# CarminLiu/ORB_SLAM2_aruco

Hardware: AMD Instinct MI355X
Metric: frames/s (ORB+ArUco extract+match, 640x480 mono) (higher is better)
Workload: dtype u8

## Files before the change

orb_slam2_aruco_amd/csrc/aruco_detector.hip:

```cpp
#include <algorithm>
#include <array>
#include <cmath>
#include <cstdlib>
#include <functional>
#include <limits>
#include <map>

#include "aruco_kernels.hpp"
#include "aruco_pose.hpp"
#include "detector_plan.hpp"
#include "host_stage.hpp"
#include "orbfe_common.hpp"
#include "orbfe_tables.inc"

using namespace orbfe;

struct ModeRun {
    const uint8_t* d_full = nullptr;
    size_t full_fstride = 0, full_step = 0;
    int full_rows = 0, full_cols = 0;
    int fixed_thr = -1;
    uint32_t* d_hist = nullptr;
    std::function<int(hipStream_t)> before_finalize;
};
// ... 10 lines not shown
struct DetectorQueues {
    hipStream_t own_stream = nullptr, aux_stream = nullptr;
    hipEvent_t ev_fork = nullptr, ev_join = nullptr;
    ~DetectorQueues()
    {
        if (own_stream) (void)hipStreamDestroy(own_stream);
        if (aux_stream) (void)hipStreamDestroy(aux_stream);
        if (ev_fork) (void)hipEventDestroy(ev_fork);
        if (ev_join) (void)hipEventDestroy(ev_join);
    }
};

struct orbfe_aruco : DetectorQueues {
    int device = 0;
    std::string dict_name;
    int nbits = 0, nb = 0, S = 0, ncodes = 0;
    hipStream_t user_aux = nullptr;
    DetectorSwitches sw;
    DetectorGeometry geo;
    int batch_cap = 0;
    DevBuf d_twork, d_trect, d_tctr;
    DevBuf d_rstate, d_lut;
    DevBuf d_segs, d_tailkeys, d_tailoff, d_small, d_hint;
    PinnedBuf pinned;
    DevBuf d_poses;
    struct Spec {
        bool pending = false, has_pose = false;
        int rows = 0, cols = 0;
        const uint8_t* host_copy = nullptr;
        size_t host_pitch = 0;
        PoseCamera cam{};
        float size = 0.f;
    } spec;
    bool last_cam_valid = false;
    PoseCamera last_cam{};
    float last_size = 0.f;
    DevBuf d_dwork, d_dctr, d_ditems, d_dhist, d_dpatch;
    bool decode_dirty = false;
    bool tail_dirty = false;
    int n_escalations = 0;
    DevBuf d_ctmlist;
    bool ct_dirty = true;
    unsigned ct_gen = 0;
    bool ct_tab_dirty = true;
    DevBuf d_ctseg, d_cthtab, d_ctelem, d_ctstate, d_ctitemsA, d_ctitemsB, d_ctnitems, d_ctcodes;
    DevBuf d_tstrips, d_ttabs, d_ttab2;
    ThresholdTables ttab;
    template <class T> static int upload(DevBuf& d, const std::vector<T>& v)
    {
        if (int rc = d.ensure(v.size() * sizeof(T))) return rc;
        if (!v.empty()) ORBFE_HIP(hipMemcpy(d.p, v.data(), v.size() * sizeof(T), hipMemcpyHostToDevice));
        return ORBFE_OK;
    }
    int ensure_threshold_tables()
    {
        if (ttab.cols == geo.cols && ttab.win == geo.win) return ORBFE_OK;
        ThresholdTables fresh = plan_threshold_tables(geo.cols, geo.win);
        ttab = ThresholdTables{};
        if (!fresh.ok) return fail(ORBFE_ERR_INVALID, "matrix-core threshold tables refused a %d-pixel row at window %d", geo.cols, geo.win);
        int rc;
        if ((rc = upload(d_tstrips, fresh.strips)) || (rc = upload(d_ttabs, fresh.tabs)) || (rc = upload(d_ttab2, fresh.tab2))) return rc;
        ttab = std::move(fresh);
        return ORBFE_OK;
    }
    bool specks_ran = false;
    DevBuf d_bitsc;
    DevBuf d_codes, d_levels, d_bits, d_pyr, d_candq, d_pool, d_kept, d_rects, d_counts, d_candidx, d_ncand,
        d_result, d_gpad;
    DevBuf d_in, d_out, d_nout;
    float error_rate = 0.0f;
    int max_corr = 0, tau = 0, nsorted = 0;
    int corner_method = 1;
    DevBuf d_scodes, d_sids, d_msrc;
    int detect_mode = 0;
    int thres_method = 0;
    int thres_value = 7;
    int n_attempts_auto_fix = 3;
    float min_size = 0.f;
    bool auto_size = false;
    float ts = 0.25f;
    bool enclosed = false;
    int tracking_min = 0;
    std::map<int, int> marker_counts;
    std::vector<orbfe_marker> prev_markers;
    int last_tracked = 0;
    int gray_bits15 = 0;
    int last_attempts = 0, last_work_rows = 0, last_work_cols = 0;
    size_t rl_static = 0;
    DevBuf d_red, d_mhist, d_masks, d_bgr, d_bits2;
    template <class Batch> int with_retries(Batch&& batch, const int32_t* counts, int nframes)
    {
        for (Contours floor = Contours::tiled;;) {
            Contours ran = Contours::none; int flags_or = 0, rc;
            if ((rc = batch(floor, &ran))) return rc;
            ORBFE_HIP(hipStreamSynchronize(own_stream));
            for (int f = 0; f < nframes; f++) flags_or |= counts[f * 4 + 2];
            if (sw.force_legacy || (floor = escalate(ran, flags_or, geo.relay_tbits != 0)) == Contours::none) return ORBFE_OK;
            n_escalations++;
        }
    }
    bool stateful() const { return thres_method == 1 || auto_size || tracking_min > 0; }
    KernelTimer timer;
    int last_nframes = 0;

    int set_dictionary(const char* name)
    {
        for (int i = 0; i < ORBFE_NDICTS; i++)
            if (!strcmp(ORBFE_DICTS[i].name, name)) {
                const orbfe_dict_entry& d = ORBFE_DICTS[i];
                if (d.nbits > 36) return fail(ORBFE_ERR_DICT, "dictionary %s: %d-bit codes are not supported", name, d.nbits);
// ... 156 lines not shown
        decode_dirty = false;
        return ORBFE_OK;
    }

    ImgView pyr_view() { return ImgView{d_pyr.as<uint8_t>(), d_pyr.as<uint8_t>(), geo.pyr_fbytes, 0}; }
    void pyramid(int first, const ImgView& src0, int B, hipStream_t st)
    {
        const ImgView pyr = pyr_view();
        const std::vector<PyrKernel> K = plan_pyramid_kernels(geo, first, (unsigned)((uintptr_t)src0.base & 15), src0.pitch, src0.fstride, sw.half_pyr);
        if (first == 1 && first < geo.npyr && (K[1] == PyrKernel::half_pyr4 || K[1] == PyrKernel::half_pyr3)) {
            const int nf = K[1] == PyrKernel::half_pyr4 ? 4 : 3, bs = 1 << nf;
            HalfPyrDst P{};
            P.base = pyr.base_w; P.fstride = geo.pyr_fbytes;
            for (int p = 1; p <= nf; p++) { P.off[p - 1] = (uint32_t)geo.levels[p].off; P.pitch[p - 1] = geo.levels[p].pitch; }
            const int bw = geo.levels[0].w / bs, nblocks = bw * (geo.levels[0].h / bs);
            if (nf == 4) hipLaunchKernelGGL(k_half_pyr<4>, dim3((nblocks + 255) / 256, B), dim3(256), 0, st, src0, P, bw, nblocks);
            else hipLaunchKernelGGL(k_half_pyr<3>, dim3((nblocks + 255) / 256, B), dim3(256), 0, st, src0, P, bw, nblocks);
            first = nf + 1;
        }
        for (int p = first; p < geo.npyr; p++) {
            const ArLevel &L = geo.levels[p], &Lp = geo.levels[p - 1];
            ImgView sv = (p == 1) ? src0 : ImgView{pyr.base + Lp.off, nullptr, geo.pyr_fbytes, Lp.pitch};
            ImgView dv{pyr.base + L.off, pyr.base_w + L.off, geo.pyr_fbytes, L.pitch};
            if (K[p] == PyrKernel::half_area4) {
                const int dw4 = (L.w + 3) / 4, nthreads = dw4 * ((L.h + 1) / 2);
                hipLaunchKernelGGL(k_half_area4, dim3((nthreads + 255) / 256, B), dim3(256), 0, st, sv, dv, dw4, L.h);
            } else if (K[p] == PyrKernel::half_area) {
                hipLaunchKernelGGL(k_half_area, dim3((L.w + 63) / 64, (L.h + 3) / 4, B), dim3(256), 0, st, sv, dv, L.w, L.h);
            } else {
                const int dw4 = (L.w + 3) / 4;
                const double scale_x = 1. / ((double)L.w / Lp.w), scale_y = 1. / ((double)L.h / Lp.h);
                hipLaunchKernelGGL(k_resize_level, dim3((dw4 + 63) / 64, (L.h + 7) / 8, B), dim3(256), 0, st, sv, dv,
                                   Lp.w, Lp.h, dw4, L.h, scale_x, scale_y, L.w);
            }
        }
    }
    template <class K> K by_window(K k5, K k7, K k11, K k15) const { return geo.win == 5 ? k5 : geo.win == 7 ? k7 : geo.win == 11 ? k11 : k15; }
    int threshold(const BatchPlan& p, const ImgView& srcW, const ImgView& src0, int fixed_thr, int B, hipStream_t s, int* enlarge_k)
    {
        for (int r_ = 0; r_ < ORBFE_REPS_ARUCO(8); r_++) {
            const int ntx = (geo.cols + 63) / 64, ntl = ntx * ((geo.rows + 63) / 64);
            const dim3 tg(ntx, (geo.rows + 63) / 64, B), tg1(xcd_grid(ntl * B));
            uint32_t* bp = d_bits.as<uint32_t>();
            if (p.thr == Thr::fixed) {
                if (enclosed) {
                    if (int rc = d_bits2.ensure(geo.bits_fu32 * 4 * B)) return rc;
                    const int k = *enlarge_k = int(std::max(3.0, 3. / 1920. * float(geo.cols))) | 1;
                    if (k / 2 > 15) return fail(ORBFE_ERR_INVALID, "detectEnclosedMarkers: frame too wide (erosion size %d)", k);
                }
                hipLaunchKernelGGL(k_fixed_threshold, dim3((geo.wpr * geo.rows + 255) / 256, B), dim3(256), 0, s, srcW, geo.cols, geo.rows, fixed_thr, enclosed ? d_bits2.as<uint32_t>() : bp, geo.bits_fu32, geo.wpr);
                if (enclosed) hipLaunchKernelGGL(k_erode_cross_xor, dim3((geo.wpr * geo.rows + 255) / 256, B), dim3(256), 0, s, d_bits2.as<uint32_t>(), bp, geo.bits_fu32, geo.wpr, geo.cols, geo.rows, *enlarge_k / 2);
            } else if (p.thr == Thr::mfma) {
                const int n2 = geo.win * geo.win, n_tstrips = (int)ttab.strips.size(), nxs = (n_tstrips + 3) / 4;
                hipLaunchKernelGGL(k_threshold_mfma, dim3(xcd_grid(nxs * B)), dim3(256), 0, s, srcW, geo.cols, geo.rows, ttab.rb, -(n2 * thres_value - n2 / 2),
                                   d_tstrips.as<ThrStrip>(), d_ttabs.as<uint4>(), d_ttab2.as<uint4>(), bp, geo.bits_fu32, geo.wpr, n_tstrips, nxs, nxs * B, n2 > 127 ? 1 : 0);
            } else if (p.thr == Thr::pyr) {
                ThrPyr P{};
                P.n = p.nfuse;
                for (int l = 1; l <= p.nfuse; l++) { P.w[l - 1] = geo.levels[l].w; P.h[l - 1] = geo.levels[l].h; P.pitch[l - 1] = geo.levels[l].pitch; P.off[l - 1] = geo.levels[l].off; }
                hipLaunchKernelGGL(by_window(k_threshold_pyr<5>, k_threshold_pyr<7>, k_threshold_pyr<11>, k_threshold_pyr<15>), tg1, dim3(256), 0, s,
                                   srcW, geo.cols, geo.rows, p.thr_kk, bp, geo.bits_fu32, geo.wpr, ntx, ntl, ntl * B, pyr_view(), P);
                if (p.nfuse && r_ == 0) pyramid(p.nfuse + 1, src0, B, s);
            } else if (geo.win <= 15) hipLaunchKernelGGL(k_adaptive_threshold<7>, tg, dim3(256), 0, s, srcW, geo.cols, geo.rows, geo.win, thres_value, 1.0 / (geo.win * geo.win), bp, geo.bits_fu32, geo.wpr);
            else hipLaunchKernelGGL(k_adaptive_threshold<15>, tg, dim3(256), 0, s, srcW, geo.cols, geo.rows, geo.win, thres_value, 1.0 / (geo.win * geo.win), bp, geo.bits_fu32, geo.wpr);
        }
        return ORBFE_OK;
    }
    int speck_pass(const BatchPlan& p, int B, hipStream_t s)
    {
        int rc;
        const size_t spk_lds = speck_lds_bytes(geo.cols);
        if (!(specks_ran = p.specks)) return ORBFE_OK;
        if ((rc = d_bitsc.ensure(geo.bits_fu32 * 4 * batch_cap)) || (rc = ensure_dyn_lds(reinterpret_cast<const void*>(k_speck_clean), spk_lds))) return rc;
        hipLaunchKernelGGL(k_speck_clean, dim3((geo.rows + SPK_ROWS - 1) / SPK_ROWS, B), dim3(SPK_THREADS), spk_lds, s, d_bits.as<uint32_t>(), geo.bits_fu32, geo.wpr,
                           geo.cols, geo.rows, d_bitsc.as<uint32_t>());
        return ORBFE_OK;
    }
    int contours_tiled(const BatchPlan& p, int B, const uint32_t* cbits, hipStream_t s)
    {
        int rc;
        const int cw = p.tile_w, ncols = (geo.cols + cw - 1) / cw, nbands = (geo.rows + 31) / 32, total_tiles = ncols * nbands * B;
        const int wave_bytes = ctw_wave_lds_bytes(cw), wlds = wave_bytes * (CTW_THREADS / 64);
        const int walk_wgs = std::max(1, std::min((total_tiles / p.tpw + CTW_THREADS / 64 - 1) / (CTW_THREADS / 64), 256 * 8));
        const size_t llds = (size_t)geo.ct_lcap * 8 + 16;
        if ((rc = ensure_dyn_lds(reinterpret_cast<const void*>(k_ct_walk), (size_t)wlds)) || (rc = ensure_dyn_lds(reinterpret_cast<const void*>(k_ct_lists), llds))) return rc;
        if (ct_dirty) ORBFE_HIP(hipMemsetAsync(d_ctstate.p, 0, (size_t)CT_STATE_INTS * 4 * B, s));
        ct_gen = (ct_gen + 1) & 0xffffu;
        if (ct_gen == 0) { ct_gen = 1; ct_tab_dirty = true; }
        if (ct_tab_dirty) { ORBFE_HIP(hipMemsetAsync(d_cthtab.p, 0, d_cthtab.bytes, s)); ct_tab_dirty = false; }
        ct_dirty = true;
        if (p.band) {
            const int nb = ((geo.rows + 31) / 32 + p.band_rows - 1) / p.band_rows;
            const size_t blds = ctb_lds_bytes(geo.cols, p.band_rows);
            if ((rc = ensure_dyn_lds(reinterpret_cast<const void*>(k_ct_band), blds))) return rc;
            hipLaunchKernelGGL(k_ct_band, dim3(nb, B), dim3(CTB_THREADS), blds, s, cbits, geo.bits_fu32, geo.wpr, geo.cols, geo.rows, 70,
                               d_lut.as<uint16_t>(), p.band_rows, d_ctmlist.as<uint32_t>(), CTB_MCAP, d_cthtab.as<unsigned long long>(), geo.ct_hbits, ct_gen,
                               d_ctseg.as<uint32_t>(), (size_t)5 * geo.ct_segcap, geo.ct_segcap, d_ctstate.as<int32_t>(), d_pool.as<uint32_t>(), geo.pool_fu32,
                               (int)geo.pool_fu32, geo.relay_kcap, d_tailkeys.as<unsigned long long>(), d_tailoff.as<int32_t>(), d_ctcodes.as<uint4>());
        } else
            hipLaunchKernelGGL(k_ct_walk, dim3(walk_wgs), dim3(CTW_THREADS), wlds, s, cbits, geo.bits_fu32, geo.wpr, geo.cols, geo.rows, 70,
                               d_lut.as<uint16_t>(), cw, ncols, nbands, total_tiles, d_cthtab.as<unsigned long long>(), geo.ct_hbits, ct_gen,
                               d_ctseg.as<uint32_t>(), (size_t)5 * geo.ct_segcap, geo.ct_segcap, d_ctstate.as<int32_t>(), d_pool.as<uint32_t>(), geo.pool_fu32,
                               (int)geo.pool_fu32, geo.relay_kcap, d_tailkeys.as<unsigned long long>(), d_tailoff.as<int32_t>(), wave_bytes,
                               d_ctcodes.as<uint4>());
        hipLaunchKernelGGL(k_ct_lists, dim3(B), dim3(geo.ct_lcap > 4096 ? 1024 : 512), llds, s, d_ctseg.as<uint32_t>(), (size_t)5 * geo.ct_segcap, geo.ct_segcap,
                           d_ctstate.as<int32_t>(), d_cthtab.as<unsigned long long>(), geo.ct_hbits, ct_gen, d_ctelem.as<unsigned long long>(), geo.ct_lcap, 70,
                           (int)geo.pool_fu32, geo.relay_kcap, d_tailkeys.as<unsigned long long>(), d_tailoff.as<int32_t>(), d_counts.as<int32_t>(),
// ... 1029 lines not shown
```

orb_slam2_aruco_amd/csrc/aruco_kernels.hip:

```cpp
#include "aruco_kernels.hpp"
#include "wave_dpp.hpp"

#ifndef ORBFE_PRIO_DET_TAIL
#define ORBFE_PRIO_DET_TAIL 0
#endif
namespace orbfe {

__device__ __forceinline__ int a_lane_prefix(unsigned long long mask)
{
    return __builtin_amdgcn_mbcnt_hi((unsigned)(mask >> 32), __builtin_amdgcn_mbcnt_lo((unsigned)mask, 0));
}

__device__ __forceinline__ uint32_t bl_dot4_a(uint32_t a, uint32_t b, uint32_t c) { return __builtin_amdgcn_udot4(a, b, c, false); }

template <int TH_MAXR>
__global__ __launch_bounds__(256) void k_adaptive_threshold(ImgView src, int W, int H, int win, int C, double scale,
                                                            uint32_t* __restrict__ bits, size_t bits_fstride, int wpr)
{
    constexpr int TH_NLD = (16 + 2 * TH_MAXR + 3) / 4;
    __shared__ uint8_t sin[16 + 2 * TH_MAXR][64 + 2 * TH_MAXR + 2];
    __shared__ uint16_t sh[16 + 2 * TH_MAXR][64];
    const int r = win >> 1;
    const int tx0 = blockIdx.x * 64, tyb = blockIdx.y * 64, f = blockIdx.z;
    const int tid = threadIdx.x, lane = tid & 63, wid = tid >> 6;
// ... 177 lines not shown
        }
    }
    if (P.n >= 1) {
        uint8_t* pf = pyr.base_w + (size_t)f * pyr.fstride;
        {
            const int j = tid >> 3, d = tid & 7;
            const uint2 a0 = *reinterpret_cast<const uint2*>(&spx[2 * j][2 * d]), a1 = *reinterpret_cast<const uint2*>(&spx[2 * j + 1][2 * d]);
            const uint32_t o = th_half4(a0, a1);
            l1[j][d] = o;
            const int y = (ty0 >> 1) + j, x = (tx0 >> 1) + 4 * d;
            if (y < P.h[0] && x < P.w[0]) *reinterpret_cast<uint32_t*>(pf + P.off[0] + (uint32_t)(__mul24(y, P.pitch[0]) + x)) = o;
        }
        if (P.n >= 2) {
            __syncthreads();
            if (tid < 64) {
                const int j = tid >> 2, d = tid & 3;
                const uint2 a0 = *reinterpret_cast<const uint2*>(&l1[2 * j][2 * d]), a1 = *reinterpret_cast<const uint2*>(&l1[2 * j + 1][2 * d]);
                const uint32_t o = th_half4(a0, a1);
                l2[j][d] = o;
                const int y = (ty0 >> 2) + j, x = (tx0 >> 2) + 4 * d;
                if (y < P.h[1] && x < P.w[1]) *reinterpret_cast<uint32_t*>(pf + P.off[1] + (uint32_t)(__mul24(y, P.pitch[1]) + x)) = o;
            }
        }
        if (P.n >= 3) {
            __syncthreads();
            if (tid < 16) {
                const int j = tid >> 1, d = tid & 1;
                const uint2 a0 = *reinterpret_cast<const uint2*>(&l2[2 * j][2 * d]), a1 = *reinterpret_cast<const uint2*>(&l2[2 * j + 1][2 * d]);
                const uint32_t o = th_half4(a0, a1);
                l3[j][d] = o;
                const int y = (ty0 >> 3) + j, x = (tx0 >> 3) + 4 * d;
                if (y < P.h[2] && x < P.w[2]) *reinterpret_cast<uint32_t*>(pf + P.off[2] + (uint32_t)(__mul24(y, P.pitch[2]) + x)) = o;
            }
        }
        if (P.n >= 4) {
            __syncthreads();
            if (tid < 4) {
                const int j = tid;
                const uint2 a0 = *reinterpret_cast<const uint2*>(&l3[2 * j][0]), a1 = *reinterpret_cast<const uint2*>(&l3[2 * j + 1][0]);
                const uint32_t o = th_half4(a0, a1);
                const int y = (ty0 >> 4) + j, x = tx0 >> 4;
                if (y < P.h[3] && x < P.w[3]) *reinterpret_cast<uint32_t*>(pf + P.off[3] + (uint32_t)(__mul24(y, P.pitch[3]) + x)) = o;
            }
        }
    }
}
template __global__ void k_threshold_pyr<5>(ImgView, int, int, uint32_t, uint32_t*, size_t, int, int, int, int, ImgView, ThrPyr);
template __global__ void k_threshold_pyr<7>(ImgView, int, int, uint32_t, uint32_t*, size_t, int, int, int, int, ImgView, ThrPyr);
template __global__ void k_threshold_pyr<11>(ImgView, int, int, uint32_t, uint32_t*, size_t, int, int, int, int, ImgView, ThrPyr);
template __global__ void k_threshold_pyr<15>(ImgView, int, int, uint32_t, uint32_t*, size_t, int, int, int, int, ImgView, ThrPyr);

typedef int tm_v4i __attribute__((ext_vector_type(4)));
typedef int tm_v16i __attribute__((ext_vector_type(16)));
__global__ __launch_bounds__(256) void k_threshold_mfma(ImgView src, int W, int H, int rb , int kinit,
                                                        const ThrStrip* __restrict__ strips, const uint4* __restrict__ tabs,
                                                        const uint4* __restrict__ tab2, uint32_t* __restrict__ bits, size_t bits_fstride,
                                                        int wpr, int nstrips, int nx, int total, int two_centre)
{
    const int lane = threadIdx.x & 63, wid = threadIdx.x >> 6;
    int bx, f;
    if (!xcd_remap(nx, total, bx, f)) return;
    const int si = bx * 4 + wid;
    if (si >= nstrips) return;
    const ThrStrip S = strips[si];
    const int r = lane & 31, half = lane >> 5;
    const uint8_t* img = src.base + (size_t)f * src.fstride;
    const tm_v4i Ba = __builtin_bit_cast(tm_v4i, tabs[(size_t)S.tab * 64 + lane]), Bb = __builtin_bit_cast(tm_v4i, tabs[(size_t)(S.tab + 1) * 64 + lane]);
    const tm_v4i Ia = __builtin_bit_cast(tm_v4i, tabs[(size_t)(S.tab + 2) * 64 + lane]), Ib = __builtin_bit_cast(tm_v4i, tabs[(size_t)(S.tab + 3) * 64 + lane]);
    const tm_v4i V2a = __builtin_bit_cast(tm_v4i, tab2[lane]), V2b = __builtin_bit_cast(tm_v4i, tab2[64 + lane]);
    const tm_v4i C2a = __builtin_bit_cast(tm_v4i, tab2[128 + lane]), C2b = __builtin_bit_cast(tm_v4i, tab2[192 + lane]);
    const tm_v4i C3a = __builtin_bit_cast(tm_v4i, tab2[256 + lane]), C3b = __builtin_bit_cast(tm_v4i, tab2[320 + lane]);
    const uint32_t ca = (uint32_t)(half ? S.c1 : S.c0), cb = (uint32_t)S.c2;
    typedef uint32_t tm_u32x4 __attribute__((ext_vector_type(4)));
    typedef tm_u32x4 tm_u32x4_unaligned __attribute__((aligned(1)));
    const int nblk = ((H + 31) >> 5) + 1;
    auto load_rows = [&](int j, tm_u32x4& pa, tm_u32x4& pb) {
        const uint32_t ro = (uint32_t)__mul24(min(max(32 * j - rb + r, 0), H - 1), src.pitch);
        pa = *reinterpret_cast<const tm_u32x4_unaligned*>(img + (ro + ca));
        pb = *reinterpret_cast<const tm_u32x4_unaligned*>(img + (ro + cb));
    };
    tm_u32x4 na, nb;
    load_rows(0, na, nb);
    const tm_v16i c128 = {128, 128, 128, 128, 128, 128, 128, 128, 128, 128, 128, 128, 128, 128, 128, 128};
    const tm_v16i ckin = {kinit, kinit, kinit, kinit, kinit, kinit, kinit, kinit, kinit, kinit, kinit, kinit, kinit, kinit, kinit, kinit};
    const tm_v16i czero = {0, 0, 0, 0, 0, 0, 0, 0, 0, 0, 0, 0, 0, 0, 0, 0};
    tm_v4i ph = {0, 0, 0, 0}, pl = {0, 0, 0, 0}, pc = {0, 0, 0, 0};
    const uint32_t valid = (S.x0 + 32 <= W) ? 0xffffffffu : ((1u << (W - S.x0)) - 1u);
    uint32_t* brow = bits + (size_t)f * bits_fstride + (S.x0 >> 5);
    for (int j = 0; j < nblk; j++) {
        const tm_u32x4 qa = na, qb = nb;
        if (j + 1 < nblk) load_rows(j + 1, na, nb);
        constexpr uint32_t SGN = 0x80808080u;
        const tm_v4i A1a = {(int)(qa.x ^ SGN), (int)(qa.y ^ SGN), (int)(qa.z ^ SGN), (int)(qa.w ^ SGN)};
        const tm_v4i A1b = {(int)(qb.x ^ SGN), (int)(qb.y ^ SGN), (int)(qb.z ^ SGN), (int)(qb.w ^ SGN)};
        tm_v16i acc = __builtin_amdgcn_mfma_i32_32x32x32_i8(A1a, Ba, c128, 0, 0, 0);
        tm_v16i sel = __builtin_amdgcn_mfma_i32_32x32x32_i8(A1a, Ia, czero, 0, 0, 0);
        acc = __builtin_amdgcn_mfma_i32_32x32x32_i8(A1b, Bb, acc, 0, 0, 0);
        sel = __builtin_amdgcn_mfma_i32_32x32x32_i8(A1b, Ib, sel, 0, 0, 0);
        tm_v4i nh, nl, nc;
#pragma unroll
        for (int q = 0; q < 4; q++) {
            const uint32_t a0 = (uint32_t)acc[4 * q], a1 = (uint32_t)acc[4 * q + 1], a2 = (uint32_t)acc[4 * q + 2], a3 = (uint32_t)acc[4 * q + 3];
            nh[q] = (int)(__builtin_amdgcn_perm(a1, a0, 0x0c0c0501u) | __builtin_amdgcn_perm(a3, a2, 0x05010c0cu));
            nl[q] = (int)((__builtin_amdgcn_perm(a1, a0, 0x0c0c0400u) | __builtin_amdgcn_perm(a3, a2, 0x04000c0cu)) ^ SGN);
            const uint32_t c0 = (uint32_t)sel[4 * q], c1 = (uint32_t)sel[4 * q + 1], c2 = (uint32_t)sel[4 * q + 2], c3 = (uint32_t)sel[4 * q + 3];
            nc[q] = (int)(__builtin_amdgcn_perm(c1, c0, 0x0c0c0400u) | __builtin_amdgcn_perm(c3, c2, 0x04000c0cu));
        }
        if (j >= 1) {
            tm_v16i ah = __builtin_amdgcn_mfma_i32_32x32x32_i8(ph, V2a, czero, 0, 0, 0);
            tm_v16i al = __builtin_amdgcn_mfma_i32_32x32x32_i8(pl, V2a, ckin, 0, 0, 0);
            ah = __builtin_amdgcn_mfma_i32_32x32x32_i8(nh, V2b, ah, 0, 0, 0);
            al = __builtin_amdgcn_mfma_i32_32x32x32_i8(nl, V2b, al, 0, 0, 0);
            al = __builtin_amdgcn_mfma_i32_32x32x32_i8(pc, C2a, al, 0, 0, 0);
            al = __builtin_amdgcn_mfma_i32_32x32x32_i8(nc, C2b, al, 0, 0, 0);
            if (two_centre) {
                al = __builtin_amdgcn_mfma_i32_32x32x32_i8(pc, C3a, al, 0, 0, 0);
                al = __builtin_amdgcn_mfma_i32_32x32x32_i8(nc, C3b, al, 0, 0, 0);
            }
            uint32_t wbits = 0;
#pragma unroll
            for (int q = 0; q < 4; q++) {
                uint32_t t4[4];
#pragma unroll
                for (int k = 0; k < 4; k++) t4[k] = ((uint32_t)ah[4 * q + k] << 8) + (uint32_t)al[4 * q + k];
                const uint32_t sg = (__builtin_amdgcn_perm(t4[1], t4[0], 0x0c0c0703u) | __builtin_amdgcn_perm(t4[3], t4[2], 0x07030c0cu)) & SGN;
                const uint32_t nib = (sg * 0x00204081u) >> 28;
                wbits |= nib << (8 * q);
            }
            wbits <<= 4 * half;
            wbits |= (uint32_t)__shfl_xor((int)wbits, 32);
            const int y = 32 * (j - 1) + r;
            if (half == 0 && y < H) brow[(uint32_t)__mul24(y, wpr)] = ~wbits & valid;
        }
        ph = nh; pl = nl; pc = nc;
    }
}

template <int WW, int HH>
__device__ __forceinline__ void speck_pass_lds(uint32_t* P, uint32_t* Fm, uint32_t* Sm, uint32_t* An, int NR, int PWS, int tid)
{
    const int n = NR * PWS;
    const float inv_pws = 1.0f / (float)PWS;
    for (int i = tid; i < n; i += SPK_THREADS) {
        const int r = (int)(((float)i + 0.5f) * inv_pws), j = i - __mul24(r, PWS);
        uint32_t f = 0, sd = 0;
        if (j + 1 < PWS) speck_row_masks<WW>(P[i], P[i + 1], &f, &sd);
        Fm[i] = f; Sm[i] = sd;
    }
    __syncthreads();
    for (int i = tid; i < n; i += SPK_THREADS) {
        const int r = (int)(((float)i + 0.5f) * inv_pws);
        uint32_t a = 0;
        if (r + HH + 1 < NR) {
            uint32_t occ = Fm[i] | Fm[i + (HH + 1) * PWS];
#pragma unroll
            for (int k = 1; k <= HH; k++) occ |= Sm[i + k * PWS];
            a = ~occ;
        }
        An[i] = a;
    }
    __syncthreads();
    for (int i = tid; i < n; i += SPK_THREADS) {
        const int r = (int)(((float)i + 0.5f) * inv_pws), j = i - __mul24(r, PWS);
        if (r < HH) continue;
        uint32_t e = 0, el = 0;
#pragma unroll
        for (int dy = 1; dy <= HH; dy++) {
            e |= An[i - dy * PWS];
            if (j) el |= An[i - dy * PWS - 1];
        }
        P[i] &= ~speck_dilate<WW>(e, el);
    }
    __syncthreads();
}

__global__ __launch_bounds__(SPK_THREADS) void k_speck_clean(const uint32_t* __restrict__ bits, size_t bits_fstride, int wpr_g, int W, int H,
                                                             uint32_t* __restrict__ out)
{
    extern __shared__ __align__(16) uint32_t spk_smem[];
    constexpr int RCH = ORBFE_SPECK_REACH, NR = SPK_ROWS + 2 * RCH;
    const int tid = threadIdx.x, f = blockIdx.y, y0 = blockIdx.x * SPK_ROWS;
    const int pw = (W + 2 + 31) >> 5, PWS = pw + 1, n = NR * PWS;
    uint32_t* P = spk_smem;
    uint32_t* Fm = P + n;
    uint32_t* Sm = Fm + n;
    uint32_t* An = Sm + n;
    const uint32_t* gb = bits + (size_t)f * bits_fstride;
    const float inv_pws = 1.0f / (float)PWS;
    for (int i = tid; i < n; i += SPK_THREADS) {
// ... 2358 lines not shown
```

orb_slam2_aruco_amd/csrc/aruco_kernels.hpp:

```cpp
#pragma once
#include <hip/hip_runtime.h>
#include <stdint.h>

#include "aruco_trace.hpp"
#include "detector_plan.hpp"
#include "orb_kernels.hpp"

namespace orbfe {

#define AR_MAX_RECTS 256

struct ArKept {
    int off, len;
    short vx[4], vy[4];
};
struct ArRect {
    float c[4][2];
    int off, len;
};

template <int TH_MAXR>
__global__ void k_adaptive_threshold(ImgView src, int W, int H, int win, int C, double scale, uint32_t* bits,
                                     size_t bits_fstride, int wpr);
__global__ void k_threshold_mfma(ImgView src, int W, int H, int rb, int kinit, const ThrStrip* strips, const uint4* tabs, const uint4* tab2,
                                 uint32_t* bits, size_t bits_fstride, int wpr, int nstrips, int nx, int total, int two_centre);
struct ThrPyr { int n; int w[4], h[4], pitch[4]; long long off[4]; };
template <int WIN>
__global__ void k_threshold_pyr(ImgView src, int W, int H, uint32_t kk, uint32_t* bits, size_t bits_fstride, int wpr, int ntx, int ntiles,
                                int total, ImgView pyr, ThrPyr P);
#ifndef ORBFE_CAND_FILTER
#define ORBFE_CAND_FILTER 1
#endif
__global__ void k_speck_clean(const uint32_t* bits, size_t bits_fstride, int wpr_g, int W, int H, uint32_t* out);
__global__ void k_half_area(ImgView src, ImgView dst, int dw, int dh);
__global__ void k_half_area4(ImgView src, ImgView dst, int dw4, int dh);
struct HalfPyrDst { uint8_t* base; size_t fstride; uint32_t off[4]; int pitch[4]; };
template <int NF> __global__ void k_half_pyr(ImgView src, HalfPyrDst P, int bw, int nblocks);
template <bool LDS_BITS>
__global__ void k_contours_t(const uint32_t* gbits, size_t bits_fstride, int wpr_g, int W, int H, int lds_bits_words,
                           int min_len, uint32_t* candq, size_t candq_fstride, int candq_cap, uint32_t* pool,
                           size_t pool_fstride, int pool_cap, ArKept* kept_out, int kept_cap, ArRect* rects_out,
                           int rect_cap, int32_t* counts, uint32_t* gpadded, size_t gpadded_fstride, int only_flagged);

struct RelaySeg {
    uint32_t nxt;
    uint32_t len;
    uint32_t minoff;
    uint32_t stg;
    uint32_t mn;
};
__global__ void k_contours_relay(const uint32_t* gbits, size_t bits_fstride, int wpr_g, int W, int H,
                                 int lds_bits_words, int min_len, int kshift, int tbits, RelaySeg* segs, uint32_t* pool,
                                 size_t pool_fstride, int pool_cap, ArKept* kept_out, int kept_cap, int kcap,
                                 unsigned long long* tail_keys, int32_t* tail_off, int32_t* counts, int32_t* hint, uint4* small_g, int32_t* rstate, int small_elsewhere, const uint16_t* lut_g, int f0, uint32_t* candq_g, size_t candq_fstride);
__global__ void k_contours_relay8(const uint32_t* gbits, size_t bits_fstride, int wpr_g, int W, int H,
                                 int lds_bits_words, int min_len, int kshift, int tbits, RelaySeg* segs, uint32_t* pool,
                                 size_t pool_fstride, int pool_cap, ArKept* kept_out, int kept_cap, int kcap,
                                 unsigned long long* tail_keys, int32_t* tail_off, int32_t* counts, int32_t* hint, uint4* small_g, int32_t* rstate, int small_elsewhere, const uint16_t* lut_g, int f0, uint32_t* candq_g, size_t candq_fstride);
__global__ void k_contours_relay_wide(const uint32_t* gbits, size_t bits_fstride, int wpr_g, int W, int H,
                                 int lds_bits_words, int min_len, int kshift, int tbits, RelaySeg* segs, uint32_t* pool,
                                 size_t pool_fstride, int pool_cap, ArKept* kept_out, int kept_cap, int kcap,
                                 unsigned long long* tail_keys, int32_t* tail_off, int32_t* counts, int32_t* hint, uint4* small_g, int32_t* rstate, int small_elsewhere, const uint16_t* lut_g, int f0, uint32_t* candq_g, size_t candq_fstride);
__global__ void k_contours_relay8g(const uint32_t* gbits, size_t bits_fstride, int wpr_g, int W, int H,
                                 int lds_bits_words, int min_len, int kshift, int tbits, RelaySeg* segs, uint32_t* pool,
                                 size_t pool_fstride, int pool_cap, ArKept* kept_out, int kept_cap, int kcap,
                                 unsigned long long* tail_keys, int32_t* tail_off, int32_t* counts, int32_t* hint, uint4* small_g, int32_t* rstate,
                                 uint32_t* gpad, size_t gpad_fstride, const uint16_t* lut_g, int f0);
__global__ void k_relay_lut(uint16_t* lut);
__global__ void k_contours_small(const uint32_t* gbits, size_t bits_fstride, int wpr_g, int W, int H, int min_len, const uint16_t* lut_g,
                                 int32_t* rstate, uint32_t* pool, size_t pool_fstride, int pool_cap, int kcap, unsigned long long* tail_keys,
                                 int32_t* tail_off, int32_t* counts);
__global__ void k_tail_prep(const unsigned long long* tail_keys, const int32_t* tail_off, int kcap, const int32_t* counts, uint4* work, size_t work_half,
                            int32_t* ctr);
__global__ void k_tail_approx(int kcap, const uint4* work, size_t work_half, const int32_t* ctr, const uint32_t* pool, size_t pool_fstride, ArKept* kept_out,
                              int kept_cap, uint8_t* rectflag, int pts);
__global__ void k_tail_finish(int kcap, const uint8_t* rectflag, const ArKept* kept_out, int kept_cap, ArRect* rects_out, int rect_cap,
// ... 121 lines not shown
```

orb_slam2_aruco_amd/csrc/detector_plan.hpp:

```cpp
#pragma once
#include <stddef.h>
#include <stdint.h>

#include <algorithm>
#include <cstdarg>
#include <cstdio>
#include <cstdlib>
#include <vector>

#include "../../include/orbfe.h"
#include "aruco_trace.hpp"
#include "input_layout.hpp"

namespace orbfe {

#define AR_MAX_KEPT 1024
#define AR_MAX_KEPT_BIG 4096
#define RL_KCAP AR_MAX_KEPT
#define CTW_MAX_CW 480
#define AR_FLAG_KEPT 2
#define AR_FLAG_POOL 4
#define AR_CAPACITY_FLAGS (AR_FLAG_KEPT | AR_FLAG_POOL)
#define RL_FLAG_TABLE 32
#define RL_FLAG_BUG 64
// ... 111 lines not shown
    const bool large = (size_t)rows * cols > (size_t)640 * 480 * 3 / 2;
    if (g.lds_bits_words && large && relay_lds_bytes(g.lds_bits_words, RL_KCAP, 13) + rl_static <= 160 * 1024) g.relay_tbits = 13;
    else if (g.lds_bits_words && relay_lds_bytes(g.lds_bits_words, RL_KCAP, 12) + rl_static <= 160 * 1024) g.relay_tbits = 12;
    g.relay_global = !g.relay_tbits && relay_lds_bytes(0, AR_MAX_KEPT_BIG, 13) + rl_static <= 160 * 1024;
    if (g.relay_global) { g.relay_tbits = 13; g.relay_kcap = AR_MAX_KEPT_BIG; }
    int sc = 4096;
    while (sc < rows * cols / 32 && sc < 65536) sc <<= 1;
    g.ct_segcap = std::min(sc, 65535);
    g.ct_hbits = 1;
    while ((1 << g.ct_hbits) < 2 * sc) g.ct_hbits++;
    g.ct_lcap = std::min(g.ct_segcap, lcap_override > 0 ? lcap_override : large ? 16384 : 4096);
    g.ct_items_per_frame = std::max(4096, g.ct_segcap / 4);
    return g;
}

enum class PyrKernel : int { none = 0, half_pyr4, half_pyr3, half_area4, half_area, resize_level };

inline std::vector<PyrKernel> plan_pyramid_kernels(const DetectorGeometry& geo, int first, unsigned src_align, int src_pitch, size_t src_fstride, bool half_pyr)
{
    std::vector<PyrKernel> k((size_t)std::max(geo.npyr, 0), PyrKernel::none);
    if (first == 1 && half_pyr)
        for (int nf = 4; nf >= 3 && first == 1; nf--) {
            const int bs = 1 << nf, al0 = bs == 16 ? 16 : 8;
            bool ok = geo.npyr > nf && geo.levels[0].w % bs == 0 && geo.levels[0].h % bs == 0 && src_pitch % al0 == 0 && src_fstride % al0 == 0 &&
                      (src_align & (unsigned)(al0 - 1)) == 0 && geo.pyr_fbytes % 8 == 0;
            for (int p = 1; ok && p <= nf; p++) {
                const int al = bs >> p;
                ok = geo.lvl_exact[p] && geo.levels[p].w == geo.levels[0].w >> p && geo.levels[p].h == geo.levels[0].h >> p && geo.levels[p].pitch % al == 0 &&
                     geo.levels[p].off % al == 0 && geo.levels[p].pitch >= geo.levels[p].w;
            }
            if (!ok) continue;
            for (int p = 1; p <= nf; p++) k[(size_t)p] = nf == 4 ? PyrKernel::half_pyr4 : PyrKernel::half_pyr3;
            first = nf + 1;
        }
    for (int p = std::max(first, 1); p < geo.npyr; p++) {
        const ArLevel &L = geo.levels[(size_t)p], &Lp = geo.levels[(size_t)p - 1];
        const bool own = p > 1;
        const int spitch = own ? Lp.pitch : src_pitch;
        const size_t sfstride = own ? geo.pyr_fbytes : src_fstride;
        const unsigned salign = own ? (unsigned)(Lp.off & 15) : src_align;
        if (!geo.lvl_exact[(size_t)p]) k[(size_t)p] = PyrKernel::resize_level;
        else if (spitch % 8 == 0 && sfstride % 8 == 0 && (salign & 7) == 0 && L.pitch % 4 == 0 && L.pitch >= 4 * ((L.w + 3) / 4)) k[(size_t)p] = PyrKernel::half_area4;
        else k[(size_t)p] = PyrKernel::half_area;
    }
    return k;
}

struct ThrStrip { int x0, c0, c1, c2, tab; };

struct ThresholdTables {
    int cols = 0, win = 0;
    bool ok = false;
    int rb = 0;
    std::vector<ThrStrip> strips;
    std::vector<uint8_t> tabs, tab2;
};

inline bool threshold_tables_apply(int cols, int win) { return win / 2 <= 7 && cols >= 48; }

inline ThresholdTables plan_threshold_tables(int cols, int win)
{
    ThresholdTables t;
    t.cols = cols; t.win = win;
    const int R = win / 2, n2 = win * win, W = cols, rb = R <= 3 ? 4 : 8;
    if (!threshold_tables_apply(cols, win)) return t;
    t.tabs.reserve((size_t)(W + 31) / 32 * 4096);
    for (int X = 0; X < W; X += 32) {
        ThrStrip S{};
        S.x0 = X; S.tab = (int)(t.tabs.size() / 1024);
        auto cl = [&](int c) { return std::min(std::max(c, 0), W - 16); };
        S.c0 = cl(X - rb); S.c1 = cl(X - rb + 16); S.c2 = cl(X - rb + 32);
        const int cs[3] = {S.c0, S.c1, S.c2};
        auto owner = [&](int x) {
            for (int pz = 0; pz < 3; pz++)
                if (x >= cs[pz] && x < cs[pz] + 16) return pz;
            return -1;
        };
        const size_t base = t.tabs.size();
        t.tabs.resize(base + 4096, 0);
        auto entry = [&](int m, int n, int piece, int x) -> uint8_t& {
            return t.tabs[base + (size_t)(m + (piece == 2)) * 1024 + (size_t)(n + 32 * (piece == 1)) * 16 + (x - cs[piece])];
        };
        for (int n = 0; n < 32 && X + n < W; n++) {
            for (int u = -R; u <= R; u++) {
                const int x = std::min(std::max(X + n + u, 0), W - 1), piece = owner(x);
                if (piece < 0) return t;
                entry(0, n, piece, x) += 1;
            }
            entry(2, n, owner(X + n), X + n) = 1;
        }
        t.strips.push_back(S);
    }
    t.tab2.assign(6144, 0);
    const int cw1 = n2 <= 127 ? n2 : 113, cw2 = n2 - cw1;
    for (int m = 0; m < 6; m++)
        for (int lane = 0; lane < 64; lane++) {
            const int n = lane & 31, half = lane >> 5;
            for (int i = 0; i < 16; i++) {
                const int q = 4 * half + (i & 3) + 8 * (i >> 2);
                const int d = ((m & 1) ? 32 : 0) + q - rb - n;
                int v = 0;
                if (m < 2) v = (d >= -R && d <= R) ? 1 : 0;
                else v = d == 0 ? -(m < 4 ? cw1 : cw2) : 0;
                t.tab2[(size_t)m * 1024 + (size_t)lane * 16 + i] = (uint8_t)(int8_t)v;
            }
        }
    t.rb = rb;
    t.ok = true;
    return t;
}

struct DetectorSwitches {
    int tiled = -1;
    int banded = -1;
    int band_rows = 0;
    int tile_w = 0;
    int tpw = 0;
    int lcap = 0;
    int specks = -1;
    bool specks_inkernel = false;
    bool relay_wide = true;
    int small_separate = -1;
    bool thr_mfma = true;
    bool thr_mfma_auto = true;
    bool thr_pyr = true;
    bool half_pyr = true;
    bool force_legacy = false;
    bool big_mode = false;
};

typedef const char* (*EnvLookup)(const char* name);
inline void read_detector_env(DetectorSwitches& sw, EnvLookup env)
{
    auto num = [&](const char* name, int unset) { const char* v = env(name); return v ? atoi(v) : unset; };
    auto tri = [&](const char* name, int unset) { const char* v = env(name); return v ? (atoi(v) ? 1 : 0) : unset; };
    sw.relay_wide = num("ORBFE_ARUCO_RELAY_WIDE", 1) != 0;
    sw.small_separate = num("ORBFE_ARUCO_SMALL_SEPARATE", sw.small_separate);
    sw.tiled = tri("ORBFE_ARUCO_TILED", sw.tiled);
    sw.banded = tri("ORBFE_ARUCO_BANDED", sw.banded);
    sw.band_rows = num("ORBFE_ARUCO_BAND_ROWS", sw.band_rows);
    sw.tile_w = num("ORBFE_ARUCO_TILE_W", sw.tile_w);
    sw.tpw = num("ORBFE_ARUCO_TPW", sw.tpw);
    sw.lcap = num("ORBFE_ARUCO_LCAP", sw.lcap);
    if (const char* v = env("ORBFE_ARUCO_SPECKS")) { sw.specks = atoi(v) == 1; sw.specks_inkernel = atoi(v) == 2; }
}

enum class Contours : int8_t { tiled, relay, walker, big, none };
enum class Thr : int8_t { fixed, mfma, pyr, box };
enum class Relay : int8_t { relay, relay8, wide, relay8g };

inline Contours escalate(Contours ran, int flags_or, bool relay_ok)
{
    const bool was_tiled = ran == Contours::tiled;
    if (was_tiled && (flags_or & (AR_CAPACITY_FLAGS | RL_FALLBACK_FLAGS)) && relay_ok) return Contours::relay;
    return ran != Contours::big && (flags_or & (AR_CAPACITY_FLAGS | (was_tiled ? RL_FALLBACK_FLAGS : 0))) ? Contours::big : Contours::none;
}

struct BatchMode {
    bool adaptive = true, reduced = false;
    int thres_value = 7;
};

struct BatchPlan {
    Thr thr = Thr::box; uint32_t thr_kk = 0;
// ... 41 lines not shown
```

Baseline: 269,200.

## Fold threshold bias into MFMA tables and specialize kernel on window remainder

Folds the +128 sign-offset and the threshold constant into a spare column of the weight tables. The first MFMA can then start from a zero accumulator, and the second starts from a compile-time constant instead of broadcast vector registers. The kernel is templated on the window radius, with a waves-per-eu occupancy hint, so the two-centre branch is resolved at compile time. The row loop is unrolled by two with ping-pong buffers so the carried plane registers need no copies. In exchange there is more code, multiple kernel instantiations, and a device synchronize whenever the tables are rebuilt.

New measurement: 270,900 (median of 2 runs). No clear change (+0.6%).

```diff
diff --git a/orb_slam2_aruco_amd/csrc/aruco_detector.hip b/orb_slam2_aruco_amd/csrc/aruco_detector.hip
--- a/orb_slam2_aruco_amd/csrc/aruco_detector.hip
+++ b/orb_slam2_aruco_amd/csrc/aruco_detector.hip
@@ -86,10 +86,14 @@
         if (!v.empty()) ORBFE_HIP(hipMemcpy(d.p, v.data(), v.size() * sizeof(T), hipMemcpyHostToDevice));
         return ORBFE_OK;
     }
+    int thr_kinit() const { const int n2 = geo.win * geo.win; return -(n2 * thres_value - n2 / 2); }
     int ensure_threshold_tables()
     {
-        if (ttab.cols == geo.cols && ttab.win == geo.win) return ORBFE_OK;
+        const ThresholdStart st = plan_threshold_start(geo.win, thr_kinit());
+        if (ttab.cols == geo.cols && ttab.win == geo.win && ttab.c1 == st.c1) return ORBFE_OK;
         ThresholdTables fresh = plan_threshold_tables(geo.cols, geo.win);
+        if (fresh.ok) fold_threshold_start(fresh, st.c1);
+        if (ttab.ok) ORBFE_HIP(hipDeviceSynchronize());
         ttab = ThresholdTables{};
         if (!fresh.ok) return fail(ORBFE_ERR_INVALID, "matrix-core threshold tables refused a %d-pixel row at window %d", geo.cols, geo.win);
         int rc;
@@ -352,7 +356,19 @@
                 if (enclosed) hipLaunchKernelGGL(k_erode_cross_xor, dim3((geo.wpr * geo.rows + 255) / 256, B), dim3(256), 0, s, d_bits2.as<uint32_t>(), bp, geo.bits_fu32, geo.wpr, geo.cols, geo.rows, *enlarge_k / 2);
             } else if (p.thr == Thr::mfma) {
                 const int n2 = geo.win * geo.win, n_tstrips = (int)ttab.strips.size(), nxs = (n_tstrips + 3) / 4;
-                hipLaunchKernelGGL(k_threshold_mfma, dim3(xcd_grid(nxs * B)), dim3(256), 0, s, srcW, geo.cols, geo.rows, ttab.rb, -(n2 * thres_value - n2 / 2),
+                const int krem = plan_threshold_start(geo.win, thr_kinit()).krem;
+                auto kern = k_threshold_mfma<-1>;
+                switch (krem) {
+                case 1: kern = k_threshold_mfma<1>; break;
+                case 2: kern = k_threshold_mfma<2>; break;
+                case 3: kern = k_threshold_mfma<3>; break;
+                case 4: kern = k_threshold_mfma<4>; break;
+                case 5: kern = k_threshold_mfma<5>; break;
+                case 6: kern = k_threshold_mfma<6>; break;
+                case 7: kern = k_threshold_mfma<7>; break;
+                default: break;
+                }
+                hipLaunchKernelGGL(kern, dim3(xcd_grid(nxs * B)), dim3(256), 0, s, srcW, geo.cols, geo.rows, ttab.rb, thr_kinit(),
                                    d_tstrips.as<ThrStrip>(), d_ttabs.as<uint4>(), d_ttab2.as<uint4>(), bp, geo.bits_fu32, geo.wpr, n_tstrips, nxs, nxs * B, n2 > 127 ? 1 : 0);
             } else if (p.thr == Thr::pyr) {
                 ThrPyr P{};
diff --git a/orb_slam2_aruco_amd/csrc/aruco_kernels.hip b/orb_slam2_aruco_amd/csrc/aruco_kernels.hip
--- a/orb_slam2_aruco_amd/csrc/aruco_kernels.hip
+++ b/orb_slam2_aruco_amd/csrc/aruco_kernels.hip
@@ -253,7 +253,11 @@
 
 typedef int tm_v4i __attribute__((ext_vector_type(4)));
 typedef int tm_v16i __attribute__((ext_vector_type(16)));
-__global__ __launch_bounds__(256) void k_threshold_mfma(ImgView src, int W, int H, int rb , int kinit,
+#ifndef TM_ATTR
+#define TM_ATTR __attribute__((amdgpu_waves_per_eu(KREM >= 0 ? 4 : 3, KREM >= 0 ? 4 : 3)))
+#endif
+template <int KREM>
+__global__ __launch_bounds__(256) TM_ATTR void k_threshold_mfma(ImgView src, int W, int H, int rb , int kinit,
                                                         const ThrStrip* __restrict__ strips, const uint4* __restrict__ tabs,
                                                         const uint4* __restrict__ tab2, uint32_t* __restrict__ bits, size_t bits_fstride,
                                                         int wpr, int nstrips, int nx, int total, int two_centre)
@@ -270,6 +274,7 @@
     const tm_v4i Ia = __builtin_bit_cast(tm_v4i, tabs[(size_t)(S.tab + 2) * 64 + lane]), Ib = __builtin_bit_cast(tm_v4i, tabs[(size_t)(S.tab + 3) * 64 + lane]);
     const tm_v4i V2a = __builtin_bit_cast(tm_v4i, tab2[lane]), V2b = __builtin_bit_cast(tm_v4i, tab2[64 + lane]);
     const tm_v4i C2a = __builtin_bit_cast(tm_v4i, tab2[128 + lane]), C2b = __builtin_bit_cast(tm_v4i, tab2[192 + lane]);
+    const bool two = KREM >= 0 ? KREM >= 6 : two_centre != 0;
     const tm_v4i C3a = __builtin_bit_cast(tm_v4i, tab2[256 + lane]), C3b = __builtin_bit_cast(tm_v4i, tab2[320 + lane]);
     const uint32_t ca = (uint32_t)(half ? S.c1 : S.c0), cb = (uint32_t)S.c2;
     typedef uint32_t tm_u32x4 __attribute__((ext_vector_type(4)));
@@ -280,25 +285,26 @@
         pa = *reinterpret_cast<const tm_u32x4_unaligned*>(img + (ro + ca));
         pb = *reinterpret_cast<const tm_u32x4_unaligned*>(img + (ro + cb));
     };
-    tm_u32x4 na, nb;
-    load_rows(0, na, nb);
-    const tm_v16i c128 = {128, 128, 128, 128, 128, 128, 128, 128, 128, 128, 128, 128, 128, 128, 128, 128};
-    const tm_v16i ckin = {kinit, kinit, kinit, kinit, kinit, kinit, kinit, kinit, kinit, kinit, kinit, kinit, kinit, kinit, kinit, kinit};
+    constexpr uint32_t SGN = 0x80808080u;
+    uint32_t bkeep = half ? 0u : 0xffffffffu;
+    const uint32_t bflip = half ? (uint32_t)THR_START_BYTE * 0x01010101u : SGN;
+    asm volatile("" : "+v"(bkeep));
+    constexpr int K0 = KREM >= 0 ? KREM : 0;
+    tm_v16i cstart = {K0, K0, K0, K0, K0, K0, K0, K0, K0, K0, K0, K0, K0, K0, K0, K0};
+    if (KREM < 0) {
+        cstart = tm_v16i{kinit, kinit, kinit, kinit, kinit, kinit, kinit, kinit, kinit, kinit, kinit, kinit, kinit, kinit, kinit, kinit};
+        asm volatile("" : "+v"(cstart));
+    }
     const tm_v16i czero = {0, 0, 0, 0, 0, 0, 0, 0, 0, 0, 0, 0, 0, 0, 0, 0};
-    tm_v4i ph = {0, 0, 0, 0}, pl = {0, 0, 0, 0}, pc = {0, 0, 0, 0};
     const uint32_t valid = (S.x0 + 32 <= W) ? 0xffffffffu : ((1u << (W - S.x0)) - 1u);
     uint32_t* brow = bits + (size_t)f * bits_fstride + (S.x0 >> 5);
-    for (int j = 0; j < nblk; j++) {
-        const tm_u32x4 qa = na, qb = nb;
-        if (j + 1 < nblk) load_rows(j + 1, na, nb);
-        constexpr uint32_t SGN = 0x80808080u;
+    auto planes = [&](const tm_u32x4& qa, const tm_u32x4& qb, tm_v4i& nh, tm_v4i& nl, tm_v4i& nc) {
         const tm_v4i A1a = {(int)(qa.x ^ SGN), (int)(qa.y ^ SGN), (int)(qa.z ^ SGN), (int)(qa.w ^ SGN)};
-        const tm_v4i A1b = {(int)(qb.x ^ SGN), (int)(qb.y ^ SGN), (int)(qb.z ^ SGN), (int)(qb.w ^ SGN)};
-        tm_v16i acc = __builtin_amdgcn_mfma_i32_32x32x32_i8(A1a, Ba, c128, 0, 0, 0);
+        const tm_v4i A1b = {(int)((qb.x & bkeep) ^ bflip), (int)((qb.y & bkeep) ^ bflip), (int)((qb.z & bkeep) ^ bflip), (int)((qb.w & bkeep) ^ bflip)};
+        tm_v16i acc = __builtin_amdgcn_mfma_i32_32x32x32_i8(A1a, Ba, czero, 0, 0, 0);
         tm_v16i sel = __builtin_amdgcn_mfma_i32_32x32x32_i8(A1a, Ia, czero, 0, 0, 0);
         acc = __builtin_amdgcn_mfma_i32_32x32x32_i8(A1b, Bb, acc, 0, 0, 0);
         sel = __builtin_amdgcn_mfma_i32_32x32x32_i8(A1b, Ib, sel, 0, 0, 0);
-        tm_v4i nh, nl, nc;
 #pragma unroll
         for (int q = 0; q < 4; q++) {
             const uint32_t a0 = (uint32_t)acc[4 * q], a1 = (uint32_t)acc[4 * q + 1], a2 = (uint32_t)acc[4 * q + 2], a3 = (uint32_t)acc[4 * q + 3];
@@ -307,35 +313,51 @@
             const uint32_t c0 = (uint32_t)sel[4 * q], c1 = (uint32_t)sel[4 * q + 1], c2 = (uint32_t)sel[4 * q + 2], c3 = (uint32_t)sel[4 * q + 3];
             nc[q] = (int)(__builtin_amdgcn_perm(c1, c0, 0x0c0c0400u) | __builtin_amdgcn_perm(c3, c2, 0x04000c0cu));
         }
-        if (j >= 1) {
-            tm_v16i ah = __builtin_amdgcn_mfma_i32_32x32x32_i8(ph, V2a, czero, 0, 0, 0);
-            tm_v16i al = __builtin_amdgcn_mfma_i32_32x32x32_i8(pl, V2a, ckin, 0, 0, 0);
-            ah = __builtin_amdgcn_mfma_i32_32x32x32_i8(nh, V2b, ah, 0, 0, 0);
-            al = __builtin_amdgcn_mfma_i32_32x32x32_i8(nl, V2b, al, 0, 0, 0);
-            al = __builtin_amdgcn_mfma_i32_32x32x32_i8(pc, C2a, al, 0, 0, 0);
-            al = __builtin_amdgcn_mfma_i32_32x32x32_i8(nc, C2b, al, 0, 0, 0);
-            if (two_centre) {
-                al = __builtin_amdgcn_mfma_i32_32x32x32_i8(pc, C3a, al, 0, 0, 0);
-                al = __builtin_amdgcn_mfma_i32_32x32x32_i8(nc, C3b, al, 0, 0, 0);
-            }
-            uint32_t wbits = 0;
-#pragma unroll
-            for (int q = 0; q < 4; q++) {
-                uint32_t t4[4];
-#pragma unroll
-                for (int k = 0; k < 4; k++) t4[k] = ((uint32_t)ah[4 * q + k] << 8) + (uint32_t)al[4 * q + k];
-                const uint32_t sg = (__builtin_amdgcn_perm(t4[1], t4[0], 0x0c0c0703u) | __builtin_amdgcn_perm(t4[3], t4[2], 0x07030c0cu)) & SGN;
-                const uint32_t nib = (sg * 0x00204081u) >> 28;
-                wbits |= nib << (8 * q);
-            }
-            wbits <<= 4 * half;
-            wbits |= (uint32_t)__shfl_xor((int)wbits, 32);
-            const int y = 32 * (j - 1) + r;
-            if (half == 0 && y < H) brow[(uint32_t)__mul24(y, wpr)] = ~wbits & valid;
-        }
-        ph = nh; pl = nl; pc = nc;
-    }
-}
+    };
+    auto rows_out = [&](int j, const tm_v4i& ph, const tm_v4i& pl, const tm_v4i& pc, const tm_v4i& nh, const tm_v4i& nl, const tm_v4i& nc) {
+        tm_v16i ah = __builtin_amdgcn_mfma_i32_32x32x32_i8(ph, V2a, czero, 0, 0, 0);
+        tm_v16i al = __builtin_amdgcn_mfma_i32_32x32x32_i8(pl, V2a, cstart, 0, 0, 0);
+        ah = __builtin_amdgcn_mfma_i32_32x32x32_i8(nh, V2b, ah, 0, 0, 0);
+        al = __builtin_amdgcn_mfma_i32_32x32x32_i8(nl, V2b, al, 0, 0, 0);
+        al = __builtin_amdgcn_mfma_i32_32x32x32_i8(pc, C2a, al, 0, 0, 0);
+        al = __builtin_amdgcn_mfma_i32_32x32x32_i8(nc, C2b, al, 0, 0, 0);
+        if (two) {
+            al = __builtin_amdgcn_mfma_i32_32x32x32_i8(pc, C3a, al, 0, 0, 0);
+            al = __builtin_amdgcn_mfma_i32_32x32x32_i8(nc, C3b, al, 0, 0, 0);
+        }
+        uint32_t wbits = 0;
+#pragma unroll
+        for (int q = 0; q < 4; q++) {
+            uint32_t t4[4];
+#pragma unroll
+            for (int k = 0; k < 4; k++) t4[k] = ((uint32_t)ah[4 * q + k] << 8) + (uint32_t)al[4 * q + k];
+            const uint32_t sg = (__builtin_amdgcn_perm(t4[1], t4[0], 0x0c0c0703u) | __builtin_amdgcn_perm(t4[3], t4[2], 0x07030c0cu)) & SGN;
+            const uint32_t nib = (sg * 0x00204081u) >> 28;
+            wbits |= nib << (8 * q);
+        }
+        wbits <<= 4 * half;
+        wbits |= (uint32_t)__shfl_xor((int)wbits, 32);
+        const int y = 32 * (j - 1) + r;
+        if (half == 0 && y < H) brow[(uint32_t)__mul24(y, wpr)] = ~wbits & valid;
+    };
+    tm_u32x4 ea, eb, oa, ob;
+    tm_v4i eh, el, ec, oh, ol, oc;
+    load_rows(0, ea, eb);
+    load_rows(1, oa, ob);
+    planes(ea, eb, eh, el, ec);
+    for (int j = 1; j < nblk; j += 2) {
+        if (j + 1 < nblk) load_rows(j + 1, ea, eb);
+        planes(oa, ob, oh, ol, oc);
+        rows_out(j, eh, el, ec, oh, ol, oc);
+        if (j + 1 >= nblk) break;
+        if (j + 2 < nblk) load_rows(j + 2, oa, ob);
+        planes(ea, eb, eh, el, ec);
+        rows_out(j + 1, oh, ol, oc, eh, el, ec);
+    }
+}
+#define TM_INSTANCE(K) template __global__ void k_threshold_mfma<K>(ImgView, int, int, int, int, const ThrStrip*, const uint4*, const uint4*, uint32_t*, size_t, int, int, int, int, int);
+TM_INSTANCE(-1) TM_INSTANCE(1) TM_INSTANCE(2) TM_INSTANCE(3) TM_INSTANCE(4) TM_INSTANCE(5) TM_INSTANCE(6) TM_INSTANCE(7)
+#undef TM_INSTANCE
 
 template <int WW, int HH>
 __device__ __forceinline__ void speck_pass_lds(uint32_t* P, uint32_t* Fm, uint32_t* Sm, uint32_t* An, int NR, int PWS, int tid)
diff --git a/orb_slam2_aruco_amd/csrc/aruco_kernels.hpp b/orb_slam2_aruco_amd/csrc/aruco_kernels.hpp
--- a/orb_slam2_aruco_amd/csrc/aruco_kernels.hpp
+++ b/orb_slam2_aruco_amd/csrc/aruco_kernels.hpp
@@ -22,6 +22,7 @@
 template <int TH_MAXR>
 __global__ void k_adaptive_threshold(ImgView src, int W, int H, int win, int C, double scale, uint32_t* bits,
                                      size_t bits_fstride, int wpr);
+template <int KREM>
 __global__ void k_threshold_mfma(ImgView src, int W, int H, int rb, int kinit, const ThrStrip* strips, const uint4* tabs, const uint4* tab2,
                                  uint32_t* bits, size_t bits_fstride, int wpr, int nstrips, int nx, int total, int two_centre);
 struct ThrPyr { int n; int w[4], h[4], pitch[4]; long long off[4]; };
diff --git a/orb_slam2_aruco_amd/csrc/detector_plan.hpp b/orb_slam2_aruco_amd/csrc/detector_plan.hpp
--- a/orb_slam2_aruco_amd/csrc/detector_plan.hpp
+++ b/orb_slam2_aruco_amd/csrc/detector_plan.hpp
@@ -187,6 +187,7 @@
     int cols = 0, win = 0;
     bool ok = false;
     int rb = 0;
+    int c1 = 0;
     std::vector<ThrStrip> strips;
     std::vector<uint8_t> tabs, tab2;
 };
@@ -245,6 +246,28 @@
     return t;
 }
 
+constexpr int THR_START_BYTE = 1;
+struct ThresholdStart { int c1, krem; };
+inline ThresholdStart plan_threshold_start(int win, int kinit)
+{
+    const int R = win / 2;
+    if (R >= 1 && R <= 7 && (kinit - R) % win == 0) {
+        const int c1 = 128 + (kinit - R) / win;
+        if (c1 >= -2048 && c1 <= 2032) return ThresholdStart{c1, R};
+    }
+    return ThresholdStart{128, -1};
+}
+inline void fold_threshold_start(ThresholdTables& t, int c1)
+{
+    int w[16], rest = c1;
+    for (int k = 0; k < 16; k++) { w[k] = std::min(std::max(rest, -128), 127); rest -= w[k]; }
+    for (const ThrStrip& S : t.strips)
+        for (int n = 0; n < 32; n++)
+            for (int k = 0; k < 16; k++) t.tabs[((size_t)S.tab + 1) * 1024 + (size_t)(n + 32) * 16 + k] = (uint8_t)(int8_t)w[k];
+    t.c1 = rest == 0 ? c1 : 0;
+    if (rest != 0) t.ok = false;
+}
+
 struct DetectorSwitches {
     int tiled = -1;
     int banded = -1;
```
